# cbacary/MoDeGPT

Measured on AMD Instinct MI355X. Metric: transformer layers compressed/sec (covariance+decomp+rebuild), Llama-3-8B @30%, higher is better.
Workload: dtype f64 from int8 MFMA digit planes, exact route: nine plane pairs + fp64 remainder sums, nothing truncated (error <= 5e-15 per call: fp64 rounding)

## Files before the change

### modegpt_amd/csrc/mlp.hip

```cpp
#include "common.hpp"

namespace mdg {
int gemm_f64(int64_t M, int64_t N, int64_t K, double alpha, const void* A, int a_dtype, int64_t sa_i, int64_t sa_k,
             const int64_t* a_rows, const void* B, int b_dtype, int64_t sb_k, int64_t sb_j, double beta, void* C,
             int c_dtype, int64_t ldc, int64_t batch, int64_t a_bs, int64_t b_bs, int64_t c_bs, int flags,
             hipStream_t st);
int potrf_lower(double* A, int64_t n, int64_t lda, double* inv_diag, hipStream_t st);
int potrs_lower(const double* L, int64_t n, int64_t ldl, const double* inv_diag, double* X, int64_t nrhs, int64_t ldx,
                double* ws, hipStream_t st);
size_t potrs_ws_elems(int64_t n, int64_t nrhs);
int copy_lower(const double* src, int64_t ld_src, const int64_t* idx, double* dst, int64_t ldd, int64_t n,
               double ridge, hipStream_t st);
}

using namespace mdg;

static int64_t ckk_pitch(int64_t r) { return (r + 15) / 16 * 16; }
extern "C" size_t mdg_nystrom_down_ws_bytes(int64_t n, int64_t r, int64_t d) {
  return ((size_t)r * ckk_pitch(r) + mdg_potrf_inv_diag_elems(r) + (size_t)r * d + potrs_ws_elems(r, d)) * sizeof(double);
}

static int nystrom_down(const double* C, int64_t n, int64_t ldc, const int64_t* idx, int64_t r, const void* Wd, int64_t d, int64_t ld_wd,
                        int w_dtype, double eps, void* down_out, int64_t ld_out, double* down_f64, void* ws, size_t ws_bytes,
                        void* side_stream, void* ev_fork, void* ev_join, void* stream);

extern "C" int mdg_nystrom_down(const double* C, int64_t n, int64_t ldc, const int64_t* idx, int64_t r, const void* Wd,
                                int64_t d, int64_t ld_wd, int w_dtype, double eps, void* down_out, int64_t ld_out,
                                double* down_f64, void* ws, size_t ws_bytes, void* stream) {
  return nystrom_down(C, n, ldc, idx, r, Wd, d, ld_wd, w_dtype, eps, down_out, ld_out, down_f64, ws, ws_bytes, nullptr, nullptr, nullptr, stream);
}

extern "C" int mdg_nystrom_down_overlapped(const double* C, int64_t n, int64_t ldc, const int64_t* idx, int64_t r, const void* Wd,
                                           int64_t d, int64_t ld_wd, int w_dtype, double eps, void* down_out, int64_t ld_out,
                                           double* down_f64, void* ws, size_t ws_bytes, void* side_stream, void* ev_fork, void* ev_join,
                                           void* stream) {
  MDG_CLEAR();
  MDG_CHECK_ARG(side_stream && ev_fork && ev_join && side_stream != stream,
                "mdg_nystrom_down_overlapped: needs a second stream and two events of the caller's");
  return nystrom_down(C, n, ldc, idx, r, Wd, d, ld_wd, w_dtype, eps, down_out, ld_out, down_f64, ws, ws_bytes, side_stream, ev_fork, ev_join, stream);
}

static int nystrom_down(const double* C, int64_t n, int64_t ldc, const int64_t* idx, int64_t r, const void* Wd, int64_t d, int64_t ld_wd,
                        int w_dtype, double eps, void* down_out, int64_t ld_out, double* down_f64, void* ws, size_t ws_bytes,
                        void* side_stream, void* ev_fork, void* ev_join, void* stream) {
  MDG_CLEAR();
  MDG_CHECK_ARG(C && idx && Wd && down_out, "mdg_nystrom_down: null pointer");
  MDG_CHECK_ARG(w_dtype == MDG_BF16 || w_dtype == MDG_F64, "mdg_nystrom_down: W_d must be bf16 or f64 (got %d)", w_dtype);
  MDG_CHECK_ARG(n > 0 && r > 0 && r <= n && d > 0 && ldc >= n && ld_wd >= n && ld_out >= r,
                "mdg_nystrom_down: bad sizes (n=%lld r=%lld d=%lld)", (long long)n, (long long)r, (long long)d);
  MDG_CHECK_ARG(ws && ws_bytes >= mdg_nystrom_down_ws_bytes(n, r, d), "mdg_nystrom_down: workspace %zu < required %zu",
                ws_bytes, mdg_nystrom_down_ws_bytes(n, r, d));
  hipStream_t st = (hipStream_t)stream;
  double* Ckk = (double*)ws;
  const int64_t ldk = ckk_pitch(r);
  double* inv = Ckk + (size_t)r * ldk;
  double* X = inv + mdg_potrf_inv_diag_elems(r);
  double* solve_ws = X + (size_t)r * d;
  MDG_TRY(copy_lower(C, ldc, idx, Ckk, ldk, r, eps, st));
  hipStream_t cross_st = st;
  if (side_stream) {
    cross_st = (hipStream_t)side_stream;
    MDG_HIP(hipEventRecord((hipEvent_t)ev_fork, st));
    MDG_HIP(hipStreamWaitEvent(cross_st, (hipEvent_t)ev_fork, 0));
  }
  MDG_TRY(gemm_f64(r, d, n, 1.0, C, MDG_F64, ldc, 1, idx, Wd, w_dtype, 1, ld_wd, 0.0, X, MDG_F64, d, 1, 0, 0, 0, 0, cross_st));
  if (side_stream) MDG_HIP(hipEventRecord((hipEvent_t)ev_join, cross_st));
  const int rc_potrf = potrf_lower(Ckk, r, ldk, inv, st);
  if (side_stream) MDG_HIP(hipStreamWaitEvent(st, (hipEvent_t)ev_join, 0));
  if (rc_potrf != MDG_OK) return rc_potrf;
  MDG_TRY(potrs_lower(Ckk, r, ldk, inv, X, d, d, solve_ws, st));
  if (down_f64) MDG_HIP(hipMemcpyAsync(down_f64, X, (size_t)r * d * sizeof(double), hipMemcpyDeviceToDevice, st));
  return mdg_cast_transpose_f64_bf16(X, r, d, d, down_out, ld_out, stream);
}
```

Baseline: 1.178.

## Split Nystrom down-projection into kept-block identity plus complement-column GEMM

Rather than running the full r x n by n x d GEMM over all columns, the kept-index block is handled algebraically. Its contribution C_kk·W_k becomes (C_kk+eps I)·W_k - eps·W_k, so after the solve it reduces to W_k plus a small correction, and this is applied with a transpose kernel. Only the n-r complement columns are gathered (a bitmap-plus-scan kernel finds them) and multiplied with a GEMM of reduced K. This cuts GEMM work by roughly r/n, at the cost of extra gather kernels, a single-block complement kernel, larger workspace, and a cap on n.

Result: faster. 1.194 (median of 6 runs) (+1.4%).

```diff
diff --git a/modegpt_amd/csrc/mlp.hip b/modegpt_amd/csrc/mlp.hip
--- a/modegpt_amd/csrc/mlp.hip
+++ b/modegpt_amd/csrc/mlp.hip
@@ -11,13 +11,105 @@
 size_t potrs_ws_elems(int64_t n, int64_t nrhs);
 int copy_lower(const double* src, int64_t ld_src, const int64_t* idx, double* dst, int64_t ldd, int64_t n,
                double ridge, hipStream_t st);
+
+constexpr int CPL_THREADS = 1024;
+constexpr int64_t CPL_MAX_N = (int64_t)1 << 18;
+
+__global__ __launch_bounds__(CPL_THREADS) void complement_kernel(const int64_t* idx, int64_t r, int64_t n, int64_t* R) {
+  extern __shared__ unsigned bits[];
+  __shared__ int scan[CPL_THREADS];
+  const int tid = threadIdx.x;
+  const int64_t words = (n + 31) / 32;
+  for (int64_t w = tid; w < words; w += CPL_THREADS) bits[w] = 0u;
+  __syncthreads();
+  for (int64_t i = tid; i < r; i += CPL_THREADS) {
+    const int64_t v = idx[i];
+    if (v >= 0 && v < n) atomicOr(&bits[v >> 5], 1u << (v & 31));
+  }
+  __syncthreads();
+  const int64_t chunk = (n + CPL_THREADS - 1) / CPL_THREADS;
+  const int64_t p0 = min(n, tid * chunk), p1 = min(n, p0 + chunk);
+  int cnt = 0;
+  for (int64_t p = p0; p < p1; p++) cnt += !((bits[p >> 5] >> (p & 31)) & 1u);
+  scan[tid] = cnt;
+  __syncthreads();
+  for (int off = 1; off < CPL_THREADS; off *= 2) {
+    const int add = tid >= off ? scan[tid - off] : 0;
+    __syncthreads();
+    scan[tid] += add;
+    __syncthreads();
+  }
+  int64_t o = scan[tid] - cnt;
+  for (int64_t p = p0; p < p1; p++)
+    if (!((bits[p >> 5] >> (p & 31)) & 1u)) R[o++] = p;
+}
+
+template <typename T>
+__global__ __launch_bounds__(256) void gather_cols_kernel(const T* src, int64_t ld_src, const int64_t* rows, const int64_t* cols,
+                                                          int64_t ncols, T* dst, int64_t ldd) {
+  const int64_t i = blockIdx.y;
+  const T* s = src + (rows ? rows[i] : i) * ld_src;
+  T* o = dst + i * ldd;
+  for (int64_t j = (int64_t)blockIdx.x * 256 + threadIdx.x; j < ldd; j += (int64_t)gridDim.x * 256) o[j] = j < ncols ? s[cols[j]] : T(0);
+}
+
+template <int DT>
+__global__ __launch_bounds__(256) void wk_transpose_kernel(const void* W, int64_t ldw, const int64_t* idx, int64_t r, int64_t d,
+                                                           double scale, int add, double* X, int64_t ldx, double* copy) {
+  __shared__ double t[64][65];
+  const int tid = threadIdx.x;
+  const int64_t i0 = (int64_t)blockIdx.y * 64, j0 = (int64_t)blockIdx.x * 64;
+  {
+    const int ii = tid & 63;
+    const int64_t i = i0 + ii;
+    const int64_t col = i < r ? idx[i] : 0;
+#pragma unroll 4
+    for (int s = 0; s < 16; s++) {
+      const int jj = (tid >> 6) + 4 * s;
+      const int64_t j = j0 + jj;
+      t[jj][ii] = (i < r && j < d) ? load_f64<DT>(W, j * ldw + col) : 0.;
+    }
+  }
+  __syncthreads();
+  const int jj = tid & 63;
+  const int64_t j = j0 + jj;
+  if (j >= d) return;
+#pragma unroll 4
+  for (int s = 0; s < 16; s++) {
+    const int ii = (tid >> 6) + 4 * s;
+    const int64_t i = i0 + ii;
+    if (i >= r) break;
+    double v = scale * t[jj][ii];
+    if (add) v += X[i * ldx + j];
+    X[i * ldx + j] = v;
+    if (copy) copy[i * ldx + j] = v;
+  }
+}
+
+static int wk_transpose(const void* W, int w_dtype, int64_t ldw, const int64_t* idx, int64_t r, int64_t d, double scale, int add,
+                        double* X, int64_t ldx, double* copy, hipStream_t st) {
+  dim3 grid((unsigned)ceil_div(d, 64), (unsigned)ceil_div(r, 64));
+  if (w_dtype == MDG_BF16)
+    hipLaunchKernelGGL(wk_transpose_kernel<MDG_BF16>, grid, dim3(256), 0, st, W, ldw, idx, r, d, scale, add, X, ldx, copy);
+  else
+    hipLaunchKernelGGL(wk_transpose_kernel<MDG_F64>, grid, dim3(256), 0, st, W, ldw, idx, r, d, scale, add, X, ldx, copy);
+  MDG_LAUNCH_CHECK();
+  return MDG_OK;
+}
 }
 
 using namespace mdg;
 
 static int64_t ckk_pitch(int64_t r) { return (r + 15) / 16 * 16; }
+static size_t align32(size_t e) { return (e + 31) / 32 * 32; }
+static size_t gather_elems(int64_t n, int64_t r, int64_t d) {
+  const size_t nr = (size_t)(n - r), pitch = (nr + 15) / 16 * 16;
+  return align32(nr) + align32((size_t)r * pitch) + align32((size_t)d * pitch);
+}
 extern "C" size_t mdg_nystrom_down_ws_bytes(int64_t n, int64_t r, int64_t d) {
-  return ((size_t)r * ckk_pitch(r) + mdg_potrf_inv_diag_elems(r) + (size_t)r * d + potrs_ws_elems(r, d)) * sizeof(double);
+  const size_t sw = potrs_ws_elems(r, d), gw = gather_elems(n, r, d);
+  return (32 + (size_t)r * ckk_pitch(r) + align32(mdg_potrf_inv_diag_elems(r)) + align32((size_t)r * d) + (sw > gw ? sw : gw)) *
+         sizeof(double);
 }
 
 static int nystrom_down(const double* C, int64_t n, int64_t ldc, const int64_t* idx, int64_t r, const void* Wd, int64_t d, int64_t ld_wd,
@@ -50,12 +142,17 @@
                 "mdg_nystrom_down: bad sizes (n=%lld r=%lld d=%lld)", (long long)n, (long long)r, (long long)d);
   MDG_CHECK_ARG(ws && ws_bytes >= mdg_nystrom_down_ws_bytes(n, r, d), "mdg_nystrom_down: workspace %zu < required %zu",
                 ws_bytes, mdg_nystrom_down_ws_bytes(n, r, d));
+  MDG_CHECK_ARG(n <= CPL_MAX_N, "mdg_nystrom_down: n = %lld above %lld", (long long)n, (long long)CPL_MAX_N);
   hipStream_t st = (hipStream_t)stream;
-  double* Ckk = (double*)ws;
+  double* Ckk = (double*)(((uintptr_t)ws + 255) & ~(uintptr_t)255);
   const int64_t ldk = ckk_pitch(r);
   double* inv = Ckk + (size_t)r * ldk;
-  double* X = inv + mdg_potrf_inv_diag_elems(r);
-  double* solve_ws = X + (size_t)r * d;
+  double* X = inv + align32(mdg_potrf_inv_diag_elems(r));
+  double* solve_ws = X + align32((size_t)r * d);
+  const int64_t nr = n - r, pg = (nr + 15) / 16 * 16;
+  int64_t* R = (int64_t*)solve_ws;
+  double* CkR = solve_ws + align32(nr);
+  void* WR = CkR + align32((size_t)r * pg);
   MDG_TRY(copy_lower(C, ldc, idx, Ckk, ldk, r, eps, st));
   hipStream_t cross_st = st;
   if (side_stream) {
@@ -63,12 +160,33 @@
     MDG_HIP(hipEventRecord((hipEvent_t)ev_fork, st));
     MDG_HIP(hipStreamWaitEvent(cross_st, (hipEvent_t)ev_fork, 0));
   }
-  MDG_TRY(gemm_f64(r, d, n, 1.0, C, MDG_F64, ldc, 1, idx, Wd, w_dtype, 1, ld_wd, 0.0, X, MDG_F64, d, 1, 0, 0, 0, 0, cross_st));
+  int rc = wk_transpose(Wd, w_dtype, ld_wd, idx, r, d, -eps, 0, X, d, nullptr, cross_st);
+  if (rc == MDG_OK && nr > 0) {
+    const unsigned words = (unsigned)((n + 31) / 32);
+    hipLaunchKernelGGL(complement_kernel, dim3(1), dim3(CPL_THREADS), words * sizeof(unsigned), cross_st, idx, r, n, R);
+    const unsigned gx = (unsigned)(ceil_div(nr, 256) < 64 ? ceil_div(nr, 256) : 64);
+    hipLaunchKernelGGL(gather_cols_kernel<double>, dim3(gx, (unsigned)r), dim3(256), 0, cross_st, C, ldc, idx, (const int64_t*)R, nr,
+                       CkR, pg);
+    if (w_dtype == MDG_BF16)
+      hipLaunchKernelGGL(gather_cols_kernel<bf16_t>, dim3(gx, (unsigned)d), dim3(256), 0, cross_st, (const bf16_t*)Wd, ld_wd, nullptr,
+                         (const int64_t*)R, nr, (bf16_t*)WR, pg);
+    else
+      hipLaunchKernelGGL(gather_cols_kernel<double>, dim3(gx, (unsigned)d), dim3(256), 0, cross_st, (const double*)Wd, ld_wd, nullptr,
+                         (const int64_t*)R, nr, (double*)WR, pg);
+    const hipError_t e = hipGetLastError();
+    if (e != hipSuccess) {
+      set_error("nystrom_down gathers: %s", hipGetErrorString(e));
+      rc = MDG_ERR_HIP;
+    }
+    if (rc == MDG_OK) rc = gemm_f64(r, d, pg, 1.0, CkR, MDG_F64, pg, 1, nullptr, WR, w_dtype, 1, pg, 1.0, X, MDG_F64, d, 1, 0, 0, 0, 0,
+                                    cross_st);
+  }
   if (side_stream) MDG_HIP(hipEventRecord((hipEvent_t)ev_join, cross_st));
+  if (rc != MDG_OK) return rc;
   const int rc_potrf = potrf_lower(Ckk, r, ldk, inv, st);
   if (side_stream) MDG_HIP(hipStreamWaitEvent(st, (hipEvent_t)ev_join, 0));
   if (rc_potrf != MDG_OK) return rc_potrf;
   MDG_TRY(potrs_lower(Ckk, r, ldk, inv, X, d, d, solve_ws, st));
-  if (down_f64) MDG_HIP(hipMemcpyAsync(down_f64, X, (size_t)r * d * sizeof(double), hipMemcpyDeviceToDevice, st));
+  MDG_TRY(wk_transpose(Wd, w_dtype, ld_wd, idx, r, d, 1.0, 1, X, d, down_f64, st));
   return mdg_cast_transpose_f64_bf16(X, r, d, d, down_out, ld_out, stream);
 }
```
